# hukaixuan19970627/yolov5_obb

Measured on AMD Instinct MI355X. Metric: val.py img/s (hot path: non_max_suppression_obb, bs16) + NMS ms/img @100k cand, DOTAv1.5 1024^2, 1/2/4/8 GPU, higher is better.
Workload: dtype f16; 1 GPU; DOTAv1.5 1024^2 bs16 (BASELINE metric; configs[1] thresholds): yolov5 OBB head output (16,64512,201) fp16, 4 distinct tensors rotated (cold: 1.66 GB working set) -> non_max_suppression_obb (conf .25, iou .45, multi_label, max_det 1500), val.py --task speed hot path = dt[2] of val.py; global_batch=16, anchors_per_image=64512, nc=16, detections_per_batch=3734, parallelism=dp1 (images sharded, no data-path collective)

## Files before the change

### yolov5_obb_amd/csrc/nms_small.h

```cpp
#pragma once
#include <hip/hip_runtime.h>
#include <stdint.h>

#include "geom.h"
#include "nms_core.h"
#include "nms_limits.h"
#include "obb_device.h"

namespace obb {

#ifdef OBB_SMALL_TRACE
__device__ unsigned long long g_small_trace[2048 * 16];
__device__ unsigned long long g_small_trace_tail[2048 * 4];
__device__ unsigned long long g_small_trace2[2048 * 8];
#define STRACE(kind, ...) do { if (threadIdx.x == 0 && blockIdx.x < 2048) { const unsigned long long v_[] = {__VA_ARGS__}; unsigned long long* o_ = g_small_trace + blockIdx.x * 16; o_[0] = (kind); for (int z_ = 0; z_ < (int)(sizeof(v_) / 8) && z_ < 15; z_++) o_[1 + z_] = v_[z_]; } } while (0)
#endif
constexpr int kSmallThreads = 512;
constexpr int kSmallWaves = kSmallThreads / 64;

struct SmallArgs {
  const float4* rec;
  const u64* alive;
  const int* seg_begin;
  const int* seg_end;
  int* keep_cnt;
  int64_t* keep_out;
  int* too_big;
  float thr;
  int max_keep;
  const unsigned long long* keys_sorted;
  const uint32_t* vals_sorted;
  const int* mode;
  int ncs;
  unsigned long long* pub_key;
  uint32_t* pub_val;
  long long n_pos;
  int helpers;
  const int* help_cnt;
  const int* work;
  const int* seg_np;
  int* seg_ticket;
  u64* part_main;
  u64* part_help;
  const unsigned long long* keys_in;
  const float4* cand;
  const int* cnt;
  const int* tiny;
  long long cap_img, max_nms, A;
  int nc;
  float class_offset;
  int* seg_max;
};
struct SmallFromSort { static constexpr bool kSelf = false; };
constexpr int kSmallClipWaves = 4;
constexpr int kSmallSplit1 = 128;
__host__ __device__ __forceinline__ int small_parts(int n) {
  return n <= kSmallSplit1 ? 1 : (n <= 192 ? 2 : (n <= 256 ? 4 : (n <= 320 ? 6 : 8)));
}
struct SmallNoTail {
  struct Args {};
  static __device__ __forceinline__ void run(const SmallArgs&, const Args&, unsigned char*, int) {}
};

template <class G>
__device__ __attribute__((noinline)) int small_quick(const float4* ra, const float4* rb, float thr) {
  return G::classify_quick(ra, rb, thr, true);
}

template <class G>
__device__ __attribute__((noinline)) uint32_t small_slice_bits(const float4* s_rec, int i0, int n, uint32_t arow16, float4 cq, int j, bool jv) {
  const int lane = threadIdx.x & 63;
  const int ir = i0 + (lane & 15);
  const float4 rq = s_rec[(ir < n ? ir : 0) * G::RECQ];
  uint32_t bits = 0u;
#pragma unroll
  for (int r = 0; r < 16; r++) {
    const float4 a = rdlane4(rq, r);
    const float dx = cq.x - a.x, dy = cq.y - a.y;
    const float rs = a.z + cq.z;
    const float d2 = dx * dx + dy * dy;
    const bool apart = (d2 > rs * rs) & (fminf(a.w, cq.w) >= 2.34e-9f * d2);
    const bool row_ok = ((arow16 >> r) & 1u) != 0u && i0 + r < n;
    const bool pass = !apart & jv & (j > i0 + r) & row_ok;
    bits |= pass ? (1u << r) : 0u;
  }
  return bits;
}

template <class G>
struct SmallWave {
  float scr[G::SCR * 64];
  uint32_t q0[128], q1[128], q2[128];
};

template <class G, class FRONT>
__device__ __forceinline__ int small_segment(const SmallArgs& a, unsigned char* s_raw) {
  __shared__ int s_next, s_nkept, s_qcnt[kSmallWaves], s_qhead[kSmallWaves], s_qcnt2[kSmallWaves], s_last;
  __shared__ uint32_t s_kept[kSmallMax];
  __shared__ unsigned long long s_pk[kSmallMax];
  __shared__ uint32_t s_pv[kSmallMax];
  float4* s_rec = reinterpret_cast<float4*>(s_raw);
  u64* s_mask = reinterpret_cast<u64*>(s_rec + (size_t)kSmallMax * G::RECQ);
  u64* s_alive = s_mask + (size_t)kSmallMax * kSmallWords;
  SmallWave<G>* s_wave = reinterpret_cast<SmallWave<G>*>(s_alive + 8);
  const int tid = threadIdx.x, lane = tid & 63, wv = tid >> 6;
  int seg = (int)blockIdx.x - a.helpers, part = 0, np = 1, hbase = 0;
  if (seg < 0) {
    const int h = (int)blockIdx.x;
    if (h >= *a.help_cnt) {
#ifdef OBB_SMALL_TRACE
      STRACE(1ull, (unsigned long long)wall_clock64());
#endif
      return -1;
    }
    const int e = a.work[h];
    if (e < 0) return -1;
    seg = e & 0xffffff; part = e >> 24;
  }
  if (a.helpers > 0) { const int v = a.seg_np[seg]; if ((v & 255) > 1) { np = v & 255; hbase = v >> 8; } }
#ifdef OBB_SMALL_TRACE
  unsigned long long tt[8]; int ti_ = 0, nd0 = 0, nd1 = 0, nd2 = 0, nit = 0;
  unsigned long long acc_d0 = 0, acc_d1 = 0, acc_d2 = 0, acc_draw = 0, acc_l0 = 0, acc_l1 = 0, acc_l2 = 0;
#define SSTAMP() do { tt[ti_++] = wall_clock64(); } while (0)
#else
#define SSTAMP() do {} while (0)
#endif
  SSTAMP();
  int sb, n, md_self = 0;
  if constexpr (FRONT::kSelf) {
    const int r = FRONT::template load<G>(a, seg, reinterpret_cast<float4*>(s_raw),
                                          reinterpret_cast<u64*>(reinterpret_cast<float4*>(s_raw) + (size_t)kSmallMax * G::RECQ), s_pk, s_pv, &s_next);
    n = r & 0xffff; md_self = r >> 16;
    sb = (int)((long long)(seg / a.ncs) * a.cap_img) + (seg % a.ncs) * kSmallMax;
    if (n <= 0 || n > kSmallMax) {
      if (tid == 0) { stg_agent(a.keep_cnt + seg, 0); if (n > kSmallMax) atomicMax(a.too_big, n); }
      return seg;
    }
  } else {
    sb = a.seg_begin[seg]; n = a.seg_end[seg] - sb;
    if (n <= 0) return part == 0 ? seg : -1;
    if (n > kSmallMax) { if (tid == 0 && part == 0) atomicMax(a.too_big, n); return part == 0 ? seg : -1; }
  }
  const bool pub = a.pub_key != nullptr;
  if constexpr (!FRONT::kSelf) {
    for (int t = tid; t < n * G::RECQ; t += kSmallThreads) s_rec[t] = a.rec[(size_t)sb * G::RECQ + t];
    for (int t = tid; t < n * kSmallWords; t += kSmallThreads) s_mask[t] = 0ull;
    if (pub)
      for (int t = tid; t < n; t += kSmallThreads) { s_pk[t] = a.keys_sorted[(size_t)sb + t]; s_pv[t] = a.vals_sorted[(size_t)sb + t]; }
    if (tid < kSmallWords) {
      const int w0 = (sb >> 6) + tid, sh = sb & 63;
      u64 v = a.alive[w0] >> sh;
      if (sh) v |= a.alive[w0 + 1] << (64 - sh);
      const int left = n - tid * 64;
      if (left <= 0) v = 0ull; else if (left < 64) v &= (1ull << left) - 1ull;
      s_alive[tid] = v;
    }
  }
  if (tid == 0) s_next = 0;
  __syncthreads();
  SSTAMP();
  const float thr = a.thr;
  SmallWave<G>& W = s_wave[wv];
  PairQueue Q0{W.q0, 0, 0}, Q1{W.q1, 0, 0}, Q2{W.q2, 0, 0};
  auto hit = [&](bool h, int i, int j) { if (h) atomicOr(&s_mask[i * kSmallWords + (j >> 6)], 1ull << (j & 63)); };
  auto drain2 = [&](int cnt) {
#ifdef OBB_SMALL_TRACE
    nd2++;
#endif
    wave_sync();
    bool h = false;
    int i = 0, j = 0;
    if (lane < cnt) {
      const uint32_t e = W.q2[(Q2.head + lane) & 127];
      i = (int)(e >> 16); j = (int)(e & 0xffffu);
      h = nms_stage_exact<G>(s_rec + i * G::RECQ, s_rec + j * G::RECQ, thr, W.scr + lane);
    }
    hit(h, i, j);
    Q2.head = (Q2.head + cnt) & 127; Q2.count -= cnt;
    wave_sync();
  };
  auto drain1 = [&](int cnt) {
#ifdef OBB_SMALL_TRACE
    nd1++;
#endif
    wave_sync();
    int res = 0, i = 0, j = 0;
    uint32_t e = 0;
    if (lane < cnt) {
      e = W.q1[(Q1.head + lane) & 127];
      i = (int)(e >> 16); j = (int)(e & 0xffffu);
      res = nms_stage_full<G>(s_rec + i * G::RECQ, s_rec + j * G::RECQ, thr);
    }
    hit(res == 1, i, j);
    Q1.head = (Q1.head + cnt) & 127; Q1.count -= cnt;
    Q2.push(res == 2, e);
    wave_sync();
    if (Q2.count >= 64) drain2(64);
  };
  auto drain0 = [&](int cnt) {
#ifdef OBB_SMALL_TRACE
    nd0++;
#endif
    wave_sync();
    int res = 0, i = 0, j = 0;
    uint32_t e = 0;
    if (lane < cnt) {
      e = W.q0[(Q0.head + lane) & 127];
      i = (int)(e >> 16); j = (int)(e & 0xffffu);
      res = small_quick<G>(s_rec + i * G::RECQ, s_rec + j * G::RECQ, thr);
    }
    hit(res == 1, i, j);
    Q0.head = (Q0.head + cnt) & 127; Q0.count -= cnt;
    Q1.push(res == 3, e);
    Q2.push(res == 2, e);
    wave_sync();
    if (Q2.count >= 64) drain2(64);
    if (Q1.count >= 64) drain1(64);
  };
  {
    const int nb = (n + 63) >> 6;
    const int nitems = nb * (nb + 1) / 2 * 4;
    for (;;) {
      int it = 0;
#ifdef OBB_SMALL_TRACE
      const unsigned long long tdr_ = wall_clock64();
#endif
      if (lane == 0) it = atomicAdd(&s_next, 1);
      it = __builtin_amdgcn_readfirstlane(it) * np + part;
#ifdef OBB_SMALL_TRACE
      acc_draw += wall_clock64() - tdr_;
#endif
      if (it >= nitems) break;
#ifdef OBB_SMALL_TRACE
      nit++;
#endif
      const int tile = it >> 2, quarter = it & 3;
      int ti = 0, rem = tile;
      while (rem >= nb - ti) { rem -= nb - ti; ti++; }
      const int tj = ti + rem;
      const int j = tj * 64 + lane;
      const bool jv = j < n && ((s_alive[tj] >> lane) & 1ull);
      const float4 cq = s_rec[(j < n ? j : 0) * G::RECQ];
      const int i0 = ti * 64 + quarter * 16;
      const uint32_t arow16 = (uint32_t)(s_alive[ti] >> (quarter * 16)) & 0xffffu;
      if (i0 >= n || arow16 == 0u) continue;
      uint32_t bits = small_slice_bits<G>(s_rec, i0, n, arow16, cq, j, jv);
      while (__ballot(bits != 0u)) {
        const bool has = bits != 0u;
        const int r = __builtin_ctz(bits | 0x10000u);
        Q0.push(has, ((uint32_t)(i0 + r) << 16) | (uint32_t)j);
        bits &= bits - 1u;
#ifdef OBB_SMALL_TRACE
        if (Q0.count >= 64) { const unsigned long long td_ = wall_clock64(); drain0(64); acc_d0 += wall_clock64() - td_; }
#else
        if (Q0.count >= 64) drain0(64);
#endif
      }
    }
    SSTAMP();
    for (int stage = 0; stage < 3; stage++) {
      PairQueue& Q = stage == 0 ? Q0 : (stage == 1 ? Q1 : Q2);
#ifdef OBB_SMALL_TRACE
      const unsigned long long tl_ = wall_clock64();
      struct LeftT { unsigned long long& a; unsigned long long t; __device__ ~LeftT() { a += wall_clock64() - t; } } lt_{stage == 0 ? acc_l0 : (stage == 1 ? acc_l1 : acc_l2), tl_};
#endif
      for (;;) {
        if (stage <= 1 && Q2.count > 64) drain2(64);
        if (stage == 0 && Q1.count > 64) drain1(64);
        if (lane == 0) { s_qcnt[wv] = Q.count; s_qhead[wv] = Q.head; if (stage == 1) s_qcnt2[wv] = Q2.count; }
        __syncthreads();
        if (stage == 1) {
          int t12 = 0, fit = 1;
#pragma unroll
          for (int w = 0; w < kSmallWaves; w++) { t12 += s_qcnt[w] + s_qcnt2[w]; fit &= (s_qcnt[w] + s_qcnt2[w] <= 128) ? 1 : 0; }
#ifdef OBB_SMALL_TRACE
          { int t1_ = 0; for (int w = 0; w < kSmallWaves; w++) t1_ += s_qcnt[w]; if (tid == 0 && blockIdx.x < 2048 && g_small_trace2[blockIdx.x * 8 + 7] == 0ull) g_small_trace2[blockIdx.x * 8 + 7] = 1ull + (unsigned long long)t1_ + ((unsigned long long)(t12 - t1_) << 20); }
#endif
          if (t12 <= 64 * kSmallClipWaves && fit) {
            while (Q1.count > 0) {
              wave_sync();
              const int c1 = Q1.count < 64 ? Q1.count : 64;
              const bool mv = lane < c1;
              const uint32_t e1 = mv ? W.q1[(Q1.head + lane) & 127] : 0u;
              Q1.head = (Q1.head + c1) & 127; Q1.count -= c1;
              Q2.push(mv, e1);
              wave_sync();
            }
            __syncthreads();
            break;
          }
        }
        int pre[kSmallWaves + 1];
        pre[0] = 0;
#pragma unroll
        for (int w = 0; w < kSmallWaves; w++) pre[w + 1] = pre[w] + s_qcnt[w];
        const int total = pre[kSmallWaves];
        if (total == 0) { __syncthreads(); break; }
        const int g = wv * 64 + lane;
        int res = 0, i = 0, j = 0;
        uint32_t e = 0;
        const bool busy = wv * 64 < total;
        if (busy && g < total) {
          int w = 0;
#pragma unroll
          for (int u = 1; u < kSmallWaves; u++) w += (g >= pre[u]) ? 1 : 0;
          const uint32_t* ring = stage == 0 ? s_wave[w].q0 : (stage == 1 ? s_wave[w].q1 : s_wave[w].q2);
          e = ring[(s_qhead[w] + (g - pre[w])) & 127];
          i = (int)(e >> 16); j = (int)(e & 0xffffu);
          const float4* ra = s_rec + i * G::RECQ;
          const float4* rb = s_rec + j * G::RECQ;
          if (stage == 0) res = small_quick<G>(ra, rb, thr);
          else if (stage == 1) res = nms_stage_full<G>(ra, rb, thr);
          else res = nms_stage_exact<G>(ra, rb, thr, W.scr + lane) ? 1 : 0;
        }
        hit(res == 1, i, j);
#ifdef OBB_SMALL_TRACE
        if (busy) { if (stage == 0) nd0++; else if (stage == 1) nd1++; else nd2++; }
#endif
        __syncthreads();
        {
          const int room = kSmallWaves * 64 - pre[wv];
          const int took = room <= 0 ? 0 : (room < s_qcnt[wv] ? room : s_qcnt[wv]);
          Q.head = (Q.head + took) & 127; Q.count -= took;
        }
        if (busy) {
          if (stage == 0) { Q1.push(res == 3, e); Q2.push(res == 2, e); }
          else if (stage == 1) Q2.push(res == 2, e);
          wave_sync();
        }
        __syncthreads();
      }
    }
  }
  SSTAMP();
  __syncthreads();
  if (np > 1) {
    auto part_buf = [&](int p) -> u64* {
      return p == 0 ? a.part_main + (size_t)sb * kSmallWords : a.part_help + (size_t)(hbase + p - 1) * kSmallMax * kSmallWords;
    };
    u64* mine = part_buf(part);
    for (int t = tid; t < n * kSmallWords; t += kSmallThreads) stg_agent(mine + t, s_mask[t]);
    asm volatile("s_waitcnt vmcnt(0)" ::: "memory");
    __syncthreads();
    if (tid == 0) s_last = __hip_atomic_fetch_add(a.seg_ticket + seg, 1, __ATOMIC_RELAXED, __HIP_MEMORY_SCOPE_AGENT) == np - 1 ? 1 : 0;
    __syncthreads();
    if (!s_last) {
#ifdef OBB_SMALL_TRACE
      STRACE(2ull, (unsigned long long)seg | ((unsigned long long)part << 24) | ((unsigned long long)np << 28), (unsigned long long)n, 0ull, tt[0], tt[1], tt[2], tt[3], (unsigned long long)wall_clock64(), 0ull, 0ull, (unsigned long long)nit, (unsigned long long)nd0, (unsigned long long)nd1, (unsigned long long)nd2);
#endif
      return -1;
    }
    for (int p = 0; p < np; p++) {
      if (p == part) continue;
      const u64* src = part_buf(p);
      for (int t = tid; t < n * kSmallWords; t += kSmallThreads) { const u64 v = ldg_agent(src + t); if (v) s_mask[t] |= v; }
    }
    __syncthreads();
  }
  SSTAMP();
  if (wv == 0) {
    u64 cur = lane < kSmallWords ? s_alive[lane] : 0ull;
    int k = 0;
    const int limit = a.max_keep > 0 ? a.max_keep : 0x7fffffff;
    const int nw = (n + 63) >> 6;
    for (int w = 0; w < nw && k < limit; w++) {
      u64 pending = ((u64)(uint32_t)__builtin_amdgcn_readlane((int)(cur >> 32), w) << 32) | (uint32_t)__builtin_amdgcn_readlane((int)cur, w);
      while (pending && k < limit) {
        const int b = __builtin_ctzll(pending), i = w * 64 + b;
        if (lane == 0) s_kept[k] = (uint32_t)i;
        k++;
        if (lane < kSmallWords) cur &= ~s_mask[i * kSmallWords + lane];
        pending = ((u64)(uint32_t)__builtin_amdgcn_readlane((int)(cur >> 32), w) << 32) | (uint32_t)__builtin_amdgcn_readlane((int)cur, w);
        pending = b < 63 ? (pending & (~0ull << (b + 1))) : 0ull;
      }
    }
    if (lane == 0) s_nkept = k;
  }
  __syncthreads();
  SSTAMP();
  const int nk = s_nkept;
  if (pub) {
    const int md = FRONT::kSelf ? md_self : a.mode[seg / a.ncs];
    for (int k = tid; k < nk; k += kSmallThreads) {
      const int i = (int)s_kept[k];
      const unsigned long long key = s_pk[i];
      stg_agent(a.pub_key + (size_t)sb + k, md == 1 ? ((key << 8) | (key >> 56)) : key);
      stg_agent(a.pub_val + (size_t)sb + k, s_pv[i]);
    }
    if (tid == 0) stg_agent(a.keep_cnt + seg, nk);
  } else {
    for (int k = tid; k < nk; k += kSmallThreads) a.keep_out[(size_t)sb + k] = (int64_t)(sb + (int)s_kept[k]);
    if (tid == 0) a.keep_cnt[seg] = nk;
  }
#ifdef OBB_SMALL_TRACE
  SSTAMP();
  STRACE(3ull, (unsigned long long)seg | ((unsigned long long)part << 24) | ((unsigned long long)np << 28), (unsigned long long)n, (unsigned long long)nk, tt[0], tt[1], tt[2], tt[3], tt[4], tt[5], tt[6], (unsigned long long)nit, (unsigned long long)nd0, (unsigned long long)nd1, (unsigned long long)nd2);
  if (tid == 0 && blockIdx.x < 2048) { unsigned long long* o_ = g_small_trace2 + blockIdx.x * 8; o_[0] = acc_d0; o_[1] = acc_d1; o_[2] = acc_d2; o_[3] = acc_draw; o_[4] = acc_l0; o_[5] = acc_l1; o_[6] = acc_l2; }
#endif
#undef SSTAMP
  return seg;
}

template <class G, class TAIL, class FRONT = SmallFromSort>
__global__ __launch_bounds__(kSmallThreads) void k_nms_small(SmallArgs a, typename TAIL::Args ta) {
  extern __shared__ __attribute__((aligned(16))) unsigned char s_raw[];
  const int seg = small_segment<G, FRONT>(a, s_raw);
  if (seg < 0) return;
  TAIL::run(a, ta, s_raw, seg);
}

static_assert((size_t)kSmallMax * RotGeom::RECQ * 16 + (size_t)kSmallMax * kSmallWords * 8 + 64 + sizeof(SmallWave<RotGeom>) * kSmallWaves +
              kSmallMax * 4 + kSmallMax * 12 + 256 <= 160 * 1024, "k_nms_small: LDS budget");
static_assert(kSmallMax % 64 == 0 && kSmallMax <= 65535, "k_nms_small: pair entries are (i << 16 | j)");

template <class G>
static size_t small_lds_bytes() {
  return (size_t)kSmallMax * G::RECQ * 16 + (size_t)kSmallMax * kSmallWords * 8 + 8 * 8 + sizeof(SmallWave<G>) * kSmallWaves;
}

}
```

### yolov5_obb_amd/csrc/nmsobb_impl.h

```cpp
#pragma once
#include <hip/hip_runtime.h>
#include <stdint.h>

#include "geom.h"
#include "launch_once.h"
#include "nms_core.h"
#include "nms_driver.h"
#include "nms_head.h"
#include "nms_limits.h"
#include "nms_plan.h"
#include "nms_small.h"
#include "nmsobb_front.h"
#include "obb_device.h"
#include "obb_hip.h"
#include "psrs_sort.h"
#include "segsort.h"
#include "tta_head_plan.h"
#include "ws_layout.h"

namespace obb {

constexpr int kTinyMax = 64;
constexpr long long kTinyPairs = 262144;
constexpr int kTinyParts = 32;
// ... 684 lines not shown
    }
    long long mx = 0;
    int tf = 0, big = 0;
    if (tid < 64) {
      for (int b2 = lane; b2 < ga.bs; b2 += 64) {
        const long long c = ga.cnt[b2 * kCntPad];
        if (c > mx) mx = c;
        const int t = ga.tiny[b2];
        tf |= t & kImgSmall;
        if ((t & kImgSmall) && !img_single_list(t)) tf |= 16;
      }
      if (tid == 0 && t2 == ga.bs - 1) big = ldg_agent(ga.info + 8);
    }
    if (max_det > 0 && cnt_c > max_det) cnt_c = (int)max_det;
    if (mine && myk == 0) { s_pre[myc + 1] = cnt_c; s_seg[myc] = sb_c; }
    if (tid == 0) s_pre[0] = 0;
    const int more = __syncthreads_or(cnt_c > spec ? 1 : 0);
    if (tid < 64) {
      int v[4], sum = 0, m = 0;
#pragma unroll
      for (int j = 0; j < 4; j++) { const int c = lane * 4 + j; v[j] = c < ncs ? s_pre[c + 1] : 0; sum += v[j]; m = v[j] > m ? v[j] : m; }
      int inc = sum;
#pragma unroll
      for (int d = 1; d < 64; d <<= 1) { const int t = __shfl_up(inc, d); if (lane >= d) inc += t; }
#pragma unroll
      for (int d = 32; d >= 1; d >>= 1) { const int o = __shfl_xor(m, d); m = o > m ? o : m; }
      int run = inc - sum;
#pragma unroll
      for (int j = 0; j < 4; j++) { const int c = lane * 4 + j; run += v[j]; if (c < ncs) s_pre[c + 1] = run; }
      if (lane == 0) s_maxc = m;
    }
    __syncthreads();
    const int total = s_pre[ncs], maxc = s_maxc;
    GSTAMP();
    if (tid == 0) ga.out_count[g] = (max_det > 0 && total > max_det) ? max_det : (long long)total;
    const bool single = self ? single_self != 0 : a.mode[g] == 0;
    const bool in_lds = total <= kLds;
    auto seg_of = [&](int e) -> int {
      int lo = 0, hi = ncs - 1;
      while (lo < hi) { const int mid = (lo + hi + 1) >> 1; if (s_pre[mid] <= e) lo = mid; else hi = mid - 1; }
      return lo;
    };
    if (in_lds) {
      if (mine && myk < cnt_c) { const int e = s_pre[myc] + myk; s_val[e] = val; s_key[e] = key; s_ck[e] = ((uint32_t)myc << 16) | (uint32_t)myk; }
      if (more)
        for (int e = tid; e < total; e += kSmallThreads) {
          const int c = seg_of(e), k = e - s_pre[c];
          if (k < spec) continue;
          const size_t p = (size_t)s_seg[c] + k;
          s_val[e] = ldg_agent(a.pub_val + p);
          s_key[e] = ldg_agent(a.pub_key + p);
          s_ck[e] = ((uint32_t)c << 16) | (uint32_t)k;
        }
      __syncthreads();
    }
    GSTAMP();
    int tpe = 1;
    if (!single) while (tpe < 16 && total * tpe * 2 <= kSmallThreads) tpe <<= 1;
    int top = 1;
    while (top * 2 <= maxc) top <<= 1;
    const int sub = tid & (tpe - 1), per_round = kSmallThreads / tpe, nlist = (ncs + tpe - 1) / tpe;
    for (int e0 = 0; e0 < total; e0 += per_round) {
      const int e = e0 + tid / tpe;
      const bool valid = e < total;
      int c = 0, k = 0, rank = 0;
      if (valid) {
        if (in_lds) { const uint32_t ck = s_ck[e]; c = (int)(ck >> 16); k = (int)(ck & 0xffffu); }
        else { c = seg_of(e); k = e - s_pre[c]; }
      }
      const bool writer = valid && sub == 0;
      float4 c0 = make_float4(0.f, 0.f, 0.f, 0.f), c1 = c0;
      if (writer) {
        const uint32_t slot = in_lds ? s_val[e] : ldg_agent(a.pub_val + (size_t)s_seg[c] + k);
        const size_t ci = (size_t)g * ga.cap_img + slot;
        c0 = ga.cand[ci * 2]; c1 = ga.cand[ci * 2 + 1];
      }
      GSTAMP();
      if (valid && !single) {
        if (in_lds) {
          const unsigned long long mk = s_key[e];
          for (int j0 = 0; j0 < nlist; j0 += 8) {
            int base[8], len[8], pos[8];
#pragma unroll
            for (int j = 0; j < 8; j++) {
              const int c2 = sub + (j0 + j) * tpe;
              const bool ok = c2 < ncs && c2 != c;
              base[j] = ok ? s_pre[c2] : 0;
              len[j] = ok ? s_pre[c2 + 1] - base[j] : 0;
              pos[j] = 0;
            }
            for (int st = top; st >= 1; st >>= 1) {
              unsigned long long k2[8];
#pragma unroll
              for (int j = 0; j < 8; j++) {
                const int q = pos[j] + st;
                int at = base[j] + (q <= len[j] ? q : len[j]) - 1;
                at = at < 0 ? 0 : at;
                k2[j] = s_key[at];
              }
#pragma unroll
              for (int j = 0; j < 8; j++) {
                const int q = pos[j] + st;
                const bool take = (q <= len[j]) & (k2[j] < mk);
                pos[j] = take ? q : pos[j];
              }
            }
#pragma unroll
            for (int j = 0; j < 8; j++) rank += pos[j];
          }
        } else {
          const unsigned long long mk = ldg_agent(a.pub_key + (size_t)s_seg[c] + k);
          for (int c2 = sub; c2 < ncs; c2 += tpe) {
            if (c2 == c) continue;
            int lo = 0, hi = s_pre[c2 + 1] - s_pre[c2];
            while (lo < hi) {
              const int mid = (lo + hi) >> 1;
              if (ldg_agent(a.pub_key + (size_t)s_seg[c2] + mid) < mk) lo = mid + 1; else hi = mid;
            }
            rank += lo;
          }
        }
      }
      GSTAMP();
      for (int d = 1; d < tpe; d <<= 1) rank += __shfl_xor(rank, d);
      rank += k;
#ifdef OBB_SMALL_TRACE
      asm volatile("s_waitcnt vmcnt(0)" ::: "memory");
      GSTAMP();
#endif
      if (!writer || (max_det > 0 && rank >= max_det)) continue;
      float* o = ga.out + ((size_t)g * max_det + rank) * 7;
      o[0] = c0.x; o[1] = c0.y; o[2] = c0.z; o[3] = c0.w; o[4] = c1.x; o[5] = c1.y; o[6] = c1.z;
    }
    GSTAMP();
#ifdef OBB_SMALL_TRACE
    if (tid == 0 && blockIdx.x < 2048) { unsigned long long* o_ = g_small_trace_tail + blockIdx.x * 4; o_[0] = 1ull + (unsigned long long)g; o_[1] = (unsigned long long)total; o_[2] = tt[0]; o_[3] = tt[7]; }
#endif
#undef GSTAMP
    if (tid >= 64) return;
    const int writes = __shfl(t2, 0) == ga.bs - 1;
    if (!writes) return;
#pragma unroll
    for (int d = 32; d >= 1; d >>= 1) { const long long o = __shfl_xor(mx, d); if (o > mx) mx = o; tf |= __shfl_xor(tf, d); }
    if (ga.clean_cnt != nullptr)
      for (int b2 = lane; b2 < ga.bs; b2 += 64) { ga.clean_cnt[b2 * kCntPad] = 0; ga.clean_tiny[b2] = 0; }
    if (lane == 0) {
      const int seg4 = ldg_agent(ga.info + 4);
      ga.status[0] = big ? -1 : (mx > ga.cap_img ? mx : 0);
      const long long small_seen = ((tf & kImgSmall) ? (1ll << 62) : 0ll) | ((tf & 16) ? (1ll << 61) : 0ll);
      ga.status[1] = mx | (((long long)(big > seg4 ? big : seg4) & 0x1fffffffll) << 32) | small_seen;
    }
  }
};
static_assert(SmallGather::kLdsBytes <= (size_t)kSmallMax * RotGeom::RECQ * 16 + (size_t)kSmallMax * kSmallWords * 8 + 64 + sizeof(SmallWave<RotGeom>) * kSmallWaves,
              "SmallGather: the merge lists live where the segment state was");

static inline size_t obb_state_bytes(int64_t bs) { return align_up((size_t)bs * kCntPad * 4 + (size_t)bs * 4); }

struct ObbCarve {
  float4* cand; unsigned long long *keys_a, *keys_b; uint32_t *vals_a, *vals_b; int* cnt; int *sort_begin, *sort_end;
  int *img_end, *mode, *tiny, *ticket;
  uint32_t* srs_hist;
  int* seg_size;
  int64_t* keep;
  Carve nms;
  size_t total;
};

static inline int64_t round_cap(int64_t cap_img) { return (cap_img + 63) / 64 * 64; }

static ObbCarve obb_carve(void* base, int64_t bs, int64_t cap_img, int64_t ncs, int cus) {
  cap_img = round_cap(cap_img);
  ObbCarve cv{};
  WsCursor w(base);
  const size_t n = (size_t)bs * cap_img;
  cv.cand = w.take<float4>(n * 2);
  cv.keys_a = w.take<unsigned long long>(n); cv.keys_b = w.take<unsigned long long>(n);
  cv.vals_a = w.take<uint32_t>(n); cv.vals_b = w.take<uint32_t>(n);
  cv.cnt = w.take<int>(bs * kCntPad); cv.sort_begin = w.take<int>(bs); cv.sort_end = w.take<int>(bs);
  cv.img_end = w.take<int>(bs); cv.mode = w.take<int>(bs); cv.tiny = w.take<int>(bs);
  cv.ticket = w.take<int>(16 + (size_t)(bs + 1));
  cv.seg_size = w.take<int>((size_t)bs * 256);
  cv.srs_hist = w.take<uint32_t>((size_t)bs * ((size_t)(cap_img + kSrsTile - 1) / kSrsTile) * 256);
  cv.keep = w.take<int64_t>(n);
  w.nest([&](void* b) { return (cv.nms = carve(b, (int64_t)n, bs * ncs, RotGeom::RECQ, cap_max(bs * ncs), cus)).total; });
  cv.total = w.total();
  return cv;
}

struct NmsObbCall {
  const void* pred = nullptr; const void* objcol = nullptr;
  const HeadFront* head = nullptr; const HeadFrontTta* tta = nullptr;
  int dtype = 0;
  int64_t bs = 0, A = 0, no = 0;
  float conf_thres = 0.f, iou_thres = 0.f;
  const int32_t* classes_host = nullptr; int n_classes = 0;
  int agnostic = 0, multi_label = 0;
  int64_t max_det = 0, max_nms = 0;
  float max_wh = 0.f;
  const float* extra8 = nullptr; int64_t n_extra = 0;
  int64_t cap_img = 0, expected_cand = 0;
  float* out = nullptr; int out_packed = 0; int64_t* out_count = nullptr; int64_t* status = nullptr;
  void* ws = nullptr; size_t ws_bytes = 0;
  void* state = nullptr; size_t state_bytes = 0;
  hipStream_t stream = nullptr;
};

static NmsObbCall nms_obb_call(int dtype, int64_t bs, int64_t A, int64_t no, float conf_thres, float iou_thres, const int32_t* classes_host,
                               int n_classes, int agnostic, int multi_label, int64_t max_det, int64_t max_nms, float max_wh,
                               const float* extra8, int64_t n_extra, int64_t cap_img, int64_t expected_cand, float* out, int out_packed,
                               int64_t* out_count, int64_t* status, void* ws, size_t ws_bytes, void* stream) {
  NmsObbCall c;
  c.dtype = dtype; c.bs = bs; c.A = A; c.no = no; c.conf_thres = conf_thres; c.iou_thres = iou_thres;
  c.classes_host = classes_host; c.n_classes = n_classes; c.agnostic = agnostic; c.multi_label = multi_label;
  c.max_det = max_det; c.max_nms = max_nms; c.max_wh = max_wh; c.extra8 = extra8; c.n_extra = n_extra;
  c.cap_img = cap_img; c.expected_cand = expected_cand; c.out = out; c.out_packed = out_packed ? 1 : 0; c.out_count = out_count;
  c.status = status; c.ws = ws; c.ws_bytes = ws_bytes; c.stream = (hipStream_t)stream;
  return c;
}

struct NmsObbRun {
  const NmsObbCall& c;
  int nc;
  int64_t cap_img;
  DeviceCus dc;
  ObbCarve cv;
  ObbPlan plan;
  bool kept;
  SmallHelpBlocks hb;
  long long bar16, alive16;
  DecodeArgs d;
};

static int obb_check_args(const NmsObbCall& c) {
  const int nc = (int)(c.no - 5 - 180);
  if (c.bs < 1 || c.A < 1 || nc < 1 || nc > 256 || c.max_det < 1 || c.cap_img < 1 || (!c.pred && !c.head && !c.tta) || !c.out ||
      !c.out_count || !c.status)
    return OBB_ERR_BAD_ARG;
  if (c.A * nc + c.n_extra > 0xffffffffLL || c.bs * c.cap_img > 0x7fffffffLL) return OBB_ERR_BAD_ARG;
  if (!dtype_known(c.dtype)) return OBB_ERR_BAD_ARG;
  return OBB_OK;
}

static int obb_carve_call(NmsObbRun& r) {
  const NmsObbCall& c = r.c;
  r.nc = (int)(c.no - 5 - 180);
  r.cap_img = round_cap(c.cap_img);
  r.dc = device_cus();
  r.cv = obb_carve(c.ws, c.bs, r.cap_img, c.agnostic ? 1 : r.nc, r.dc.cus);
  return ws_ok(c.ws, c.ws_bytes, r.cv.total) ? OBB_OK : OBB_ERR_WORKSPACE;
}

static int obb_plan_call(NmsObbRun& r) {
  const NmsObbCall& c = r.c;
  ObbCarve& cv = r.cv;
  ObbPlanIn pin{};
  pin.bs = c.bs; pin.A = c.A; pin.nc = r.nc; pin.agnostic = c.agnostic; pin.multi_label = c.multi_label; pin.iou_thres = c.iou_thres; pin.max_wh = c.max_wh;
  pin.n_extra = c.n_extra; pin.cap_img = r.cap_img; pin.max_nms = c.max_nms; pin.max_det = c.max_det; pin.expected_cand = c.expected_cand;
  pin.out_packed = c.out_packed; pin.hw_cus = r.dc.hw_cus; pin.cus = r.dc.cus; pin.ecap = cv.nms.ecap;
  pin.sort_tmp_bytes = cv.nms.sort_tmp_bytes; pin.ps_scratch_bytes = ps_scratch_bytes();
  r.plan = plan_nms_obb(pin, nms_env());
  r.kept = c.state != nullptr;
  if (r.kept) {
    if (!ws_ok(c.state, c.state_bytes, obb_state_bytes(c.bs))) return OBB_ERR_WORKSPACE;
    cv.cnt = (int*)c.state;
    cv.tiny = cv.cnt + c.bs * kCntPad;
  }
  r.hb = SmallHelpBlocks{};
  if (r.plan.helpers > 0) { WsCursor w(cv.nms.edges); r.hb = small_help_layout(w, r.plan.helpers, c.bs * r.plan.ncs, c.bs * r.cap_img); }
  return OBB_OK;
}

static void obb_fill_decode(NmsObbRun& r) {
  const NmsObbCall& c = r.c;
  const ObbCarve& cv = r.cv;
  DecodeArgs& d = r.d;
  d.pred = c.pred; d.objcol = c.objcol; d.A = c.A; d.no = (int)c.no; d.nc = r.nc; d.bs = (int)c.bs; d.conf_thres = c.conf_thres;
  d.multi_label = r.plan.multi_label;
  d.rows_per_thread = r.plan.rows_per_thread;
  class_mask_fill(c.classes_host, c.n_classes, d.cm.w, &d.cm.all);
  d.cap_img = r.cap_img; d.cand = cv.cand; d.keys = cv.keys_a; d.vals = cv.vals_a; d.cnt = cv.cnt; d.tiny = cv.tiny;
  d.win_lo = -0.35f * c.max_wh; d.win_hi = 0.6f * c.max_wh;
  r.alive16 = r.plan.zero_alive ? (long long)((((size_t)c.bs * r.cap_img) >> 6) + 8 + 1) / 2 : 0ll;
  r.bar16 = r.plan.zero_bar ? (long long)(cv.nms.bar_bytes / 16) : 0ll;
  d.z_ticket = nullptr; d.n_ticket = 0; d.z_bar16 = nullptr; d.n_bar16 = 0; d.z_alive16 = nullptr; d.n_alive16 = 0;
  if (r.kept) {
    d.z_ticket = cv.ticket; d.n_ticket = (int)(16 + c.bs + 1);
    d.z_bar16 = r.bar16 ? reinterpret_cast<uint4*>(cv.nms.bar) : nullptr; d.n_bar16 = r.bar16;
    d.z_alive16 = r.alive16 ? reinterpret_cast<uint4*>(cv.nms.alive) : nullptr; d.n_alive16 = r.alive16;
  }
}

static int obb_front_stage(NmsObbRun& r) {
  const NmsObbCall& c = r.c;
  const ObbCarve& cv = r.cv;
  const DecodeArgs& d = r.d;
  hipStream_t st = c.stream;
  if (!r.kept)
    k_reset_state<<<256, 256, 0, st>>>(cv.cnt, (int)(c.bs * kCntPad), cv.tiny, (int)c.bs, c.status, cv.ticket, (int)(16 + c.bs + 1),
                                       reinterpret_cast<uint4*>(cv.nms.bar), r.bar16, reinterpret_cast<uint4*>(cv.nms.alive), r.alive16);
  dim3 gd((unsigned)((c.A + kDecThreads * d.rows_per_thread - 1) / (kDecThreads * d.rows_per_thread)), (unsigned)c.bs);
  {
    ProfScope ps(PROF_DECODE, st);
    if (c.head || c.tta) {
      const int rc = c.head ? launch_decode_head(*c.head, d, c.dtype, r.dc.dev, st) : launch_decode_head_tta(*c.tta, d, c.dtype, r.dc.dev, st);
      if (rc) return rc;
    } else OBB_DISPATCH_DTYPE(c.dtype, T, k_decode<T><<<gd, kDecThreads, 0, st>>>(d));
// ... 142 lines not shown
```

Measured before the change: 158,300 img/s.

## Replace per-wave pair queues with block-wide candidate bitmask and compacted stage lists

The small-segment NMS kernel used to push candidate pairs into per-wave ring queues, draining them through the quick, full and exact stages with frequent wave syncs and a cross-wave redistribution loop. It now records candidates as a per-row bitmask in LDS, prefix-sums the popcounts across the block, and compacts them into a flat list, in chunks of rows when the list overflows. Each stage is then run block-wide over compacted lists, with survivors routed by atomic counters into a shared two-ended list. This aims to cut queue management overhead and improve lane utilisation, at the cost of extra LDS for the candidate mask and lists, more block barriers, and a two-pass structure.

```diff
diff --git a/yolov5_obb_amd/csrc/nms_small.h b/yolov5_obb_amd/csrc/nms_small.h
--- a/yolov5_obb_amd/csrc/nms_small.h
+++ b/yolov5_obb_amd/csrc/nms_small.h
@@ -53,6 +53,8 @@
 };
 struct SmallFromSort { static constexpr bool kSelf = false; };
 constexpr int kSmallClipWaves = 4;
+constexpr int kSmallList = 4096;
+constexpr int kSmallWpt = (kSmallMax * kSmallWords + kSmallThreads - 1) / kSmallThreads;
 constexpr int kSmallSplit1 = 128;
 __host__ __device__ __forceinline__ int small_parts(int n) {
   return n <= kSmallSplit1 ? 1 : (n <= 192 ? 2 : (n <= 256 ? 4 : (n <= 320 ? 6 : 8)));
@@ -88,21 +90,25 @@
 }
 
 template <class G>
-struct SmallWave {
-  float scr[G::SCR * 64];
-  uint32_t q0[128], q1[128], q2[128];
-};
+constexpr size_t small_lds_bytes() {
+  return (size_t)kSmallMax * G::RECQ * 16 + (size_t)kSmallMax * kSmallWords * 8 * 2 + 8 * 8 + (size_t)kSmallClipWaves * G::SCR * 64 * 4 +
+         (size_t)kSmallList * 4 * 2 + (size_t)(kSmallMax + 4) * 4;
+}
 
 template <class G, class FRONT>
 __device__ __forceinline__ int small_segment(const SmallArgs& a, unsigned char* s_raw) {
-  __shared__ int s_next, s_nkept, s_qcnt[kSmallWaves], s_qhead[kSmallWaves], s_qcnt2[kSmallWaves], s_last;
+  __shared__ int s_next, s_nkept, s_n1, s_n2, s_wsum[kSmallWaves], s_last;
   __shared__ uint32_t s_kept[kSmallMax];
   __shared__ unsigned long long s_pk[kSmallMax];
   __shared__ uint32_t s_pv[kSmallMax];
   float4* s_rec = reinterpret_cast<float4*>(s_raw);
   u64* s_mask = reinterpret_cast<u64*>(s_rec + (size_t)kSmallMax * G::RECQ);
   u64* s_alive = s_mask + (size_t)kSmallMax * kSmallWords;
-  SmallWave<G>* s_wave = reinterpret_cast<SmallWave<G>*>(s_alive + 8);
+  u64* s_cand = s_alive + 8;
+  float* s_scr = reinterpret_cast<float*>(s_cand + (size_t)kSmallMax * kSmallWords);
+  uint32_t* s_l0 = reinterpret_cast<uint32_t*>(s_scr + (size_t)kSmallClipWaves * G::SCR * 64);
+  uint32_t* s_l12 = s_l0 + kSmallList;
+  uint32_t* s_roff = s_l12 + kSmallList;
   const int tid = threadIdx.x, lane = tid & 63, wv = tid >> 6;
   int seg = (int)blockIdx.x - a.helpers, part = 0, np = 1, hbase = 0;
   if (seg < 0) {
@@ -119,11 +125,16 @@
   }
   if (a.helpers > 0) { const int v = a.seg_np[seg]; if ((v & 255) > 1) { np = v & 255; hbase = v >> 8; } }
 #ifdef OBB_SMALL_TRACE
-  unsigned long long tt[8]; int ti_ = 0, nd0 = 0, nd1 = 0, nd2 = 0, nit = 0;
-  unsigned long long acc_d0 = 0, acc_d1 = 0, acc_d2 = 0, acc_draw = 0, acc_l0 = 0, acc_l1 = 0, acc_l2 = 0;
+  unsigned long long tt[8]; int ti_ = 0, nit = 0, np0 = 0, np1 = 0, np2 = 0, nchunk = 0, nfull = 0;
+  unsigned long long acc_list = 0, acc_q = 0, acc_i = 0, acc_c = 0, acc_draw = 0, route0 = 0, tph = 0;
 #define SSTAMP() do { tt[ti_++] = wall_clock64(); } while (0)
+#define SPHASE(acc) do { const unsigned long long now_ = wall_clock64(); acc += now_ - tph; tph = now_; } while (0)
+#define STR(...) __VA_ARGS__
+#define STRACE2() do { if (tid == 0 && blockIdx.x < 2048) { unsigned long long* o_ = g_small_trace2 + blockIdx.x * 8; o_[0] = acc_list; o_[1] = acc_q; o_[2] = acc_i; o_[3] = acc_c; o_[4] = acc_draw; o_[5] = (unsigned long long)nchunk; o_[6] = (unsigned long long)nfull; o_[7] = route0; } } while (0)
 #else
 #define SSTAMP() do {} while (0)
+#define SPHASE(acc) do {} while (0)
+#define STR(...)
 #endif
   SSTAMP();
   int sb, n, md_self = 0;
@@ -156,84 +167,22 @@
       s_alive[tid] = v;
     }
   }
+  for (int t = tid; t < n * kSmallWords; t += kSmallThreads) s_cand[t] = 0ull;
   if (tid == 0) s_next = 0;
   __syncthreads();
   SSTAMP();
   const float thr = a.thr;
-  SmallWave<G>& W = s_wave[wv];
-  PairQueue Q0{W.q0, 0, 0}, Q1{W.q1, 0, 0}, Q2{W.q2, 0, 0};
   auto hit = [&](bool h, int i, int j) { if (h) atomicOr(&s_mask[i * kSmallWords + (j >> 6)], 1ull << (j & 63)); };
-  auto drain2 = [&](int cnt) {
-#ifdef OBB_SMALL_TRACE
-    nd2++;
-#endif
-    wave_sync();
-    bool h = false;
-    int i = 0, j = 0;
-    if (lane < cnt) {
-      const uint32_t e = W.q2[(Q2.head + lane) & 127];
-      i = (int)(e >> 16); j = (int)(e & 0xffffu);
-      h = nms_stage_exact<G>(s_rec + i * G::RECQ, s_rec + j * G::RECQ, thr, W.scr + lane);
-    }
-    hit(h, i, j);
-    Q2.head = (Q2.head + cnt) & 127; Q2.count -= cnt;
-    wave_sync();
-  };
-  auto drain1 = [&](int cnt) {
-#ifdef OBB_SMALL_TRACE
-    nd1++;
-#endif
-    wave_sync();
-    int res = 0, i = 0, j = 0;
-    uint32_t e = 0;
-    if (lane < cnt) {
-      e = W.q1[(Q1.head + lane) & 127];
-      i = (int)(e >> 16); j = (int)(e & 0xffffu);
-      res = nms_stage_full<G>(s_rec + i * G::RECQ, s_rec + j * G::RECQ, thr);
-    }
-    hit(res == 1, i, j);
-    Q1.head = (Q1.head + cnt) & 127; Q1.count -= cnt;
-    Q2.push(res == 2, e);
-    wave_sync();
-    if (Q2.count >= 64) drain2(64);
-  };
-  auto drain0 = [&](int cnt) {
-#ifdef OBB_SMALL_TRACE
-    nd0++;
-#endif
-    wave_sync();
-    int res = 0, i = 0, j = 0;
-    uint32_t e = 0;
-    if (lane < cnt) {
-      e = W.q0[(Q0.head + lane) & 127];
-      i = (int)(e >> 16); j = (int)(e & 0xffffu);
-      res = small_quick<G>(s_rec + i * G::RECQ, s_rec + j * G::RECQ, thr);
-    }
-    hit(res == 1, i, j);
-    Q0.head = (Q0.head + cnt) & 127; Q0.count -= cnt;
-    Q1.push(res == 3, e);
-    Q2.push(res == 2, e);
-    wave_sync();
-    if (Q2.count >= 64) drain2(64);
-    if (Q1.count >= 64) drain1(64);
-  };
   {
     const int nb = (n + 63) >> 6;
     const int nitems = nb * (nb + 1) / 2 * 4;
     for (;;) {
       int it = 0;
-#ifdef OBB_SMALL_TRACE
-      const unsigned long long tdr_ = wall_clock64();
-#endif
+      STR(const unsigned long long tdr_ = wall_clock64();)
       if (lane == 0) it = atomicAdd(&s_next, 1);
       it = __builtin_amdgcn_readfirstlane(it) * np + part;
-#ifdef OBB_SMALL_TRACE
-      acc_draw += wall_clock64() - tdr_;
-#endif
+      STR(acc_draw += wall_clock64() - tdr_;)
       if (it >= nitems) break;
-#ifdef OBB_SMALL_TRACE
-      nit++;
-#endif
       const int tile = it >> 2, quarter = it & 3;
       int ti = 0, rem = tile;
       while (rem >= nb - ti) { rem -= nb - ti; ti++; }
@@ -244,92 +193,135 @@
       const int i0 = ti * 64 + quarter * 16;
       const uint32_t arow16 = (uint32_t)(s_alive[ti] >> (quarter * 16)) & 0xffffu;
       if (i0 >= n || arow16 == 0u) continue;
-      uint32_t bits = small_slice_bits<G>(s_rec, i0, n, arow16, cq, j, jv);
-      while (__ballot(bits != 0u)) {
-        const bool has = bits != 0u;
-        const int r = __builtin_ctz(bits | 0x10000u);
-        Q0.push(has, ((uint32_t)(i0 + r) << 16) | (uint32_t)j);
-        bits &= bits - 1u;
-#ifdef OBB_SMALL_TRACE
-        if (Q0.count >= 64) { const unsigned long long td_ = wall_clock64(); drain0(64); acc_d0 += wall_clock64() - td_; }
-#else
-        if (Q0.count >= 64) drain0(64);
-#endif
-      }
-    }
+      STR(nit++;)
+      const uint32_t bits = small_slice_bits<G>(s_rec, i0, n, arow16, cq, j, jv);
+      u64 word = 0ull;
+#pragma unroll
+      for (int r = 0; r < 16; r++) { const u64 m = __ballot(((bits >> r) & 1u) != 0u); if (lane == r) word = m; }
+      if (lane < 16 && i0 + lane < n) s_cand[(i0 + lane) * kSmallWords + tj] = word;
+    }
+    __syncthreads();
     SSTAMP();
-    for (int stage = 0; stage < 3; stage++) {
-      PairQueue& Q = stage == 0 ? Q0 : (stage == 1 ? Q1 : Q2);
-#ifdef OBB_SMALL_TRACE
-      const unsigned long long tl_ = wall_clock64();
-      struct LeftT { unsigned long long& a; unsigned long long t; __device__ ~LeftT() { a += wall_clock64() - t; } } lt_{stage == 0 ? acc_l0 : (stage == 1 ? acc_l1 : acc_l2), tl_};
-#endif
-      for (;;) {
-        if (stage <= 1 && Q2.count > 64) drain2(64);
-        if (stage == 0 && Q1.count > 64) drain1(64);
-        if (lane == 0) { s_qcnt[wv] = Q.count; s_qhead[wv] = Q.head; if (stage == 1) s_qcnt2[wv] = Q2.count; }
-        __syncthreads();
-        if (stage == 1) {
-          int t12 = 0, fit = 1;
-#pragma unroll
-          for (int w = 0; w < kSmallWaves; w++) { t12 += s_qcnt[w] + s_qcnt2[w]; fit &= (s_qcnt[w] + s_qcnt2[w] <= 128) ? 1 : 0; }
-#ifdef OBB_SMALL_TRACE
-          { int t1_ = 0; for (int w = 0; w < kSmallWaves; w++) t1_ += s_qcnt[w]; if (tid == 0 && blockIdx.x < 2048 && g_small_trace2[blockIdx.x * 8 + 7] == 0ull) g_small_trace2[blockIdx.x * 8 + 7] = 1ull + (unsigned long long)t1_ + ((unsigned long long)(t12 - t1_) << 20); }
-#endif
-          if (t12 <= 64 * kSmallClipWaves && fit) {
-            while (Q1.count > 0) {
-              wave_sync();
-              const int c1 = Q1.count < 64 ? Q1.count : 64;
-              const bool mv = lane < c1;
-              const uint32_t e1 = mv ? W.q1[(Q1.head + lane) & 127] : 0u;
-              Q1.head = (Q1.head + c1) & 127; Q1.count -= c1;
-              Q2.push(mv, e1);
-              wave_sync();
-            }
-            __syncthreads();
-            break;
+    STR(tph = tt[ti_ - 1];)
+    const int nwords = n * kSmallWords, w0 = tid * kSmallWpt;
+    int mycnt = 0;
+#pragma unroll
+    for (int k = 0; k < kSmallWpt; k++) mycnt += w0 + k < nwords ? __popcll(s_cand[w0 + k]) : 0;
+    int incl = mycnt;
+#pragma unroll
+    for (int d = 1; d < 64; d <<= 1) { const int v = __shfl_up(incl, d); if (lane >= d) incl += v; }
+    if (lane == 63) s_wsum[wv] = incl;
+    __syncthreads();
+    int mybase = incl - mycnt, total = 0;
+#pragma unroll
+    for (int w = 0; w < kSmallWaves; w++) { const int v = s_wsum[w]; mybase += w < wv ? v : 0; total += v; }
+    const bool chunked = total > kSmallList;
+    if (chunked) {
+      int run = mybase;
+#pragma unroll
+      for (int k = 0; k < kSmallWpt; k++) {
+        const int idx = w0 + k;
+        if (idx >= nwords) break;
+        const int row = idx / kSmallWords;
+        if (idx == row * kSmallWords) s_roff[row] = (uint32_t)run;
+        run += __popcll(s_cand[idx]);
+      }
+      if (tid == 0) s_roff[n] = (uint32_t)total;
+      __syncthreads();
+    }
+    STR(np0 = total;)
+    for (int r0 = 0; r0 < n;) {
+      int r1 = n, cbase = 0, cnt0 = total;
+      if (chunked) {
+        cbase = (int)s_roff[r0];
+        int lo = r0 + 1, hi = n;
+        while (lo < hi) { const int mid = (lo + hi + 1) >> 1; if ((int)s_roff[mid] - cbase <= kSmallList) lo = mid; else hi = mid - 1; }
+        r1 = lo; cnt0 = (int)s_roff[r1] - cbase;
+      }
+      if (cnt0 == 0) break;
+      if (tid == 0) { s_n1 = 0; s_n2 = 0; }
+      {
+        int run = mybase;
+#pragma unroll
+        for (int k = 0; k < kSmallWpt; k++) {
+          const int idx = w0 + k;
+          if (idx >= nwords) break;
+          u64 w = s_cand[idx];
+          const int row = idx / kSmallWords, at = run - cbase;
+          run += __popcll(w);
+          if (row < r0 || row >= r1) continue;
+          const uint32_t e0 = ((uint32_t)row << 16) | ((uint32_t)(idx - row * kSmallWords) << 6);
+          for (int p = at; w; w &= w - 1ull) s_l0[p++] = e0 | (uint32_t)__builtin_ctzll(w);
+        }
+      }
+      __syncthreads();
+      STR(nchunk++;)
+      SPHASE(acc_list);
+      for (int p0 = wv * 64; p0 < cnt0; p0 += kSmallThreads) {
+        const int g = p0 + lane;
+        int res = 0, i = 0, j = 0;
+        uint32_t e = 0u;
+        if (g < cnt0) {
+          e = s_l0[g];
+          i = (int)(e >> 16); j = (int)(e & 0xffffu);
+          res = small_quick<G>(s_rec + i * G::RECQ, s_rec + j * G::RECQ, thr);
+        }
+        hit(res == 1, i, j);
+        const u64 m1 = __ballot(res == 3), m2 = __ballot(res == 2);
+        if (m1 | m2) {
+          int b1 = 0, b2 = 0;
+          if (lane == 0) { if (m1) b1 = atomicAdd(&s_n1, __popcll(m1)); if (m2) b2 = atomicAdd(&s_n2, __popcll(m2)); }
+          b1 = __builtin_amdgcn_readfirstlane(b1); b2 = __builtin_amdgcn_readfirstlane(b2);
+          if (res == 3) s_l12[b1 + __popcll(m1 & lanemask_lt())] = e;
+          if (res == 2) s_l12[kSmallList - 1 - (b2 + __popcll(m2 & lanemask_lt()))] = e;
+        }
+      }
+      __syncthreads();
+      SPHASE(acc_q);
+      int n1 = s_n1, n2 = s_n2;
+      STR(if (route0 == 0ull) route0 = 1ull + (unsigned long long)n1 + ((unsigned long long)n2 << 20);)
+      if (n1 + n2 > 64 * kSmallClipWaves) {
+        STR(nfull++; np1 += n1;)
+        for (int hi = n1; hi > 0; hi -= kSmallThreads) {
+          const int lo = hi > kSmallThreads ? hi - kSmallThreads : 0, g = lo + tid;
+          const uint32_t e = g < hi ? s_l12[g] : 0u;
+          __syncthreads();
+          if (lo + wv * 64 >= hi) continue;
+          const int i = (int)(e >> 16), j = (int)(e & 0xffffu);
+          int res = 0;
+          if (g < hi) res = nms_stage_full<G>(s_rec + i * G::RECQ, s_rec + j * G::RECQ, thr);
+          hit(res == 1, i, j);
+          const u64 m2 = __ballot(res == 2);
+          if (m2) {
+            int b2 = 0;
+            if (lane == 0) b2 = atomicAdd(&s_n2, __popcll(m2));
+            b2 = __builtin_amdgcn_readfirstlane(b2);
+            if (res == 2) s_l12[kSmallList - 1 - (b2 + __popcll(m2 & lanemask_lt()))] = e;
           }
         }
-        int pre[kSmallWaves + 1];
-        pre[0] = 0;
-#pragma unroll
-        for (int w = 0; w < kSmallWaves; w++) pre[w + 1] = pre[w] + s_qcnt[w];
-        const int total = pre[kSmallWaves];
-        if (total == 0) { __syncthreads(); break; }
-        const int g = wv * 64 + lane;
-        int res = 0, i = 0, j = 0;
-        uint32_t e = 0;
-        const bool busy = wv * 64 < total;
-        if (busy && g < total) {
-          int w = 0;
-#pragma unroll
-          for (int u = 1; u < kSmallWaves; u++) w += (g >= pre[u]) ? 1 : 0;
-          const uint32_t* ring = stage == 0 ? s_wave[w].q0 : (stage == 1 ? s_wave[w].q1 : s_wave[w].q2);
-          e = ring[(s_qhead[w] + (g - pre[w])) & 127];
-          i = (int)(e >> 16); j = (int)(e & 0xffffu);
-          const float4* ra = s_rec + i * G::RECQ;
-          const float4* rb = s_rec + j * G::RECQ;
-          if (stage == 0) res = small_quick<G>(ra, rb, thr);
-          else if (stage == 1) res = nms_stage_full<G>(ra, rb, thr);
-          else res = nms_stage_exact<G>(ra, rb, thr, W.scr + lane) ? 1 : 0;
+        __syncthreads();
+        n1 = 0; n2 = s_n2;
+        SPHASE(acc_i);
+      }
+      const int nclip = n1 + n2;
+      STR(np2 += nclip;)
+      if (wv < kSmallClipWaves) {
+        float* scr = s_scr + (size_t)wv * (G::SCR * 64) + lane;
+        for (int g0 = wv * 64; g0 < nclip; g0 += 64 * kSmallClipWaves) {
+          const int g = g0 + lane;
+          bool h = false;
+          int i = 0, j = 0;
+          if (g < nclip) {
+            const uint32_t e = g < n1 ? s_l12[g] : s_l12[kSmallList - 1 - (g - n1)];
+            i = (int)(e >> 16); j = (int)(e & 0xffffu);
+            h = nms_stage_exact<G>(s_rec + i * G::RECQ, s_rec + j * G::RECQ, thr, scr);
+          }
+          hit(h, i, j);
         }
-        hit(res == 1, i, j);
-#ifdef OBB_SMALL_TRACE
-        if (busy) { if (stage == 0) nd0++; else if (stage == 1) nd1++; else nd2++; }
-#endif
-        __syncthreads();
-        {
-          const int room = kSmallWaves * 64 - pre[wv];
-          const int took = room <= 0 ? 0 : (room < s_qcnt[wv] ? room : s_qcnt[wv]);
-          Q.head = (Q.head + took) & 127; Q.count -= took;
-        }
-        if (busy) {
-          if (stage == 0) { Q1.push(res == 3, e); Q2.push(res == 2, e); }
-          else if (stage == 1) Q2.push(res == 2, e);
-          wave_sync();
-        }
-        __syncthreads();
-      }
+      }
+      SPHASE(acc_c);
+      r0 = r1;
+      if (r0 < n) __syncthreads();
     }
   }
   SSTAMP();
@@ -346,7 +338,8 @@
     __syncthreads();
     if (!s_last) {
 #ifdef OBB_SMALL_TRACE
-      STRACE(2ull, (unsigned long long)seg | ((unsigned long long)part << 24) | ((unsigned long long)np << 28), (unsigned long long)n, 0ull, tt[0], tt[1], tt[2], tt[3], (unsigned long long)wall_clock64(), 0ull, 0ull, (unsigned long long)nit, (unsigned long long)nd0, (unsigned long long)nd1, (unsigned long long)nd2);
+      STRACE(2ull, (unsigned long long)seg | ((unsigned long long)part << 24) | ((unsigned long long)np << 28), (unsigned long long)n, 0ull, tt[0], tt[1], tt[2], tt[3], (unsigned long long)wall_clock64(), 0ull, 0ull, (unsigned long long)nit, (unsigned long long)np0, (unsigned long long)np1, (unsigned long long)np2);
+      STRACE2();
 #endif
       return -1;
     }
@@ -394,10 +387,13 @@
   }
 #ifdef OBB_SMALL_TRACE
   SSTAMP();
-  STRACE(3ull, (unsigned long long)seg | ((unsigned long long)part << 24) | ((unsigned long long)np << 28), (unsigned long long)n, (unsigned long long)nk, tt[0], tt[1], tt[2], tt[3], tt[4], tt[5], tt[6], (unsigned long long)nit, (unsigned long long)nd0, (unsigned long long)nd1, (unsigned long long)nd2);
-  if (tid == 0 && blockIdx.x < 2048) { unsigned long long* o_ = g_small_trace2 + blockIdx.x * 8; o_[0] = acc_d0; o_[1] = acc_d1; o_[2] = acc_d2; o_[3] = acc_draw; o_[4] = acc_l0; o_[5] = acc_l1; o_[6] = acc_l2; }
+  STRACE(3ull, (unsigned long long)seg | ((unsigned long long)part << 24) | ((unsigned long long)np << 28), (unsigned long long)n, (unsigned long long)nk, tt[0], tt[1], tt[2], tt[3], tt[4], tt[5], tt[6], (unsigned long long)nit, (unsigned long long)np0, (unsigned long long)np1, (unsigned long long)np2);
+  STRACE2();
 #endif
 #undef SSTAMP
+#undef SPHASE
+#undef STR
+#undef STRACE2
   return seg;
 }
 
@@ -409,13 +405,8 @@
   TAIL::run(a, ta, s_raw, seg);
 }
 
-static_assert((size_t)kSmallMax * RotGeom::RECQ * 16 + (size_t)kSmallMax * kSmallWords * 8 + 64 + sizeof(SmallWave<RotGeom>) * kSmallWaves +
-              kSmallMax * 4 + kSmallMax * 12 + 256 <= 160 * 1024, "k_nms_small: LDS budget");
+static_assert(small_lds_bytes<RotGeom>() + kSmallMax * 4 + kSmallMax * 12 + 256 <= 160 * 1024, "k_nms_small: LDS budget");
 static_assert(kSmallMax % 64 == 0 && kSmallMax <= 65535, "k_nms_small: pair entries are (i << 16 | j)");
-
-template <class G>
-static size_t small_lds_bytes() {
-  return (size_t)kSmallMax * G::RECQ * 16 + (size_t)kSmallMax * kSmallWords * 8 + 8 * 8 + sizeof(SmallWave<G>) * kSmallWaves;
-}
-
-}
+static_assert(kSmallList >= kSmallMax && kSmallWpt * kSmallThreads >= kSmallMax * kSmallWords, "k_nms_small: a row fits a list chunk, every candidate word has a thread");
+
+}
diff --git a/yolov5_obb_amd/csrc/nmsobb_impl.h b/yolov5_obb_amd/csrc/nmsobb_impl.h
--- a/yolov5_obb_amd/csrc/nmsobb_impl.h
+++ b/yolov5_obb_amd/csrc/nmsobb_impl.h
@@ -860,7 +860,7 @@
     }
   }
 };
-static_assert(SmallGather::kLdsBytes <= (size_t)kSmallMax * RotGeom::RECQ * 16 + (size_t)kSmallMax * kSmallWords * 8 + 64 + sizeof(SmallWave<RotGeom>) * kSmallWaves,
+static_assert(SmallGather::kLdsBytes <= small_lds_bytes<RotGeom>(),
               "SmallGather: the merge lists live where the segment state was");
 
 static inline size_t obb_state_bytes(int64_t bs) { return align_up((size_t)bs * kCntPad * 4 + (size_t)bs * 4); }
```

Result: slower. 154,800 img/s (-2.2%).
